# vitasoftAI/ImageRetrievalResearch

Measured on AMD Instinct MI355X. Metric: images/sec embed + queries/sec top-k@100k-gallery, EffNet-B3a 224^2, higher is better.
Workload: dtype bf16

## Files before the change

### imageretrievalresearch_amd/csrc/mbconv_block.hip

```cpp
#include "ops.h"

namespace mi355 {

typedef __bf16 bf16x8 __attribute__((ext_vector_type(8)));
typedef float f32x4 __attribute__((ext_vector_type(4)));
typedef unsigned u32x4 __attribute__((ext_vector_type(4)));
typedef unsigned u32x2 __attribute__((ext_vector_type(2)));

constexpr int MB_THREADS = 512;
constexpr int MB_WAVES = MB_THREADS / 64;
constexpr int MB_MAX_RD = 192;
constexpr int MB_MC = MB_WAVES * 16;

__device__ __forceinline__ float mb_lo(unsigned u) { return __uint_as_float(u << 16); }
__device__ __forceinline__ float mb_hi(unsigned u) { return __uint_as_float(u & 0xffff0000u); }

__device__ __forceinline__ void mb_lds_barrier() {
    asm volatile("s_waitcnt lgkmcnt(0)" ::: "memory");
    __builtin_amdgcn_s_barrier();
    asm volatile("" ::: "memory");
}

__host__ __device__ static inline int mb_proj_ntw(int NTp, int MTp, int NTW) {
    int best = 1, best_busy = 0;
// ... 12 lines not shown
    const int ntw = mb_proj_ntw(NTp, MTp, 3);
    if (wi != 14) return ntw;
    const int nwn = (NTp + ntw - 1) / ntw;
    int msplit = nwn <= MB_WAVES ? MB_WAVES / nwn : 1;
    if (msplit > MTp) msplit = MTp;
    if (nwn <= MB_WAVES && (MTp + msplit - 1) / msplit <= mwp) return ntw;
    return 4;
}

template <int KS> struct MbTaps {
    static constexpr int KK = KS * KS;
    static constexpr int NV = (KS / 2) * KS;
    static constexpr int NH = (KS + 1) / 2;
    static constexpr int NP = NV + NH;
    __host__ __device__ static constexpr bool vertical(int tp) { return tp < NV; }
    __host__ __device__ static constexpr int tap_a(int tp) {
        return tp < NV ? (tp / KS) * 2 * KS + tp % KS : (KS - 1) * KS + (tp - NV) * 2;
    }
    __host__ __device__ static constexpr int tap_b(int tp) {
        return tp < NV ? tap_a(tp) + KS : ((tp - NV) * 2 + 1 < KS ? tap_a(tp) + 1 : -1);
    }
};

template <int KS, int S, int WI, int MW, int MH, int NTW, int MWP, int KST, int A_IT, int ACT_E, int ACT_D>
__global__ __launch_bounds__(MB_THREADS) void k_mbconv_block(const BlockArgs a) {
    using TP = MbTaps<KS>;
    constexpr int MC = MB_MC;
    constexpr int PAD = KS / 2;
    constexpr int NP = TP::NP;
    constexpr int EW = WI + 2 * PAD;
    constexpr int WO = (WI + 2 * PAD - KS) / S + 1;
    constexpr int TR = WO <= 8 ? 2 : 1;
    constexpr int RP = (TR == 2 && S == 1) ? ((EW + 7) & ~7) : EW;
    static_assert(WO <= 16, "depthwise tile geometry");
    constexpr bool PROJ_WHOLE = WI == 7 && NTW == 2;
    constexpr int KC = WI == 7 ? 256 : 128;
    constexpr int ALD = KC + 16;
    extern __shared__ __attribute__((aligned(16))) unsigned char mb_smem[];

    const int tid = threadIdx.x, lane = tid & 63;
    const int wave = __builtin_amdgcn_readfirstlane(tid >> 6);
    const int fr = lane & 15, fq = lane >> 4, fk = fq * 8;
    const int b = blockIdx.x;
    const int P = a.H * a.W, MT = (P + 15) >> 4, XLD = a.XLD;
    const int EH = a.H + 2 * PAD;
    const int EP = (EH + (TR == 2 ? S : 0)) * RP + 8;
    const int Pout = a.Ho * a.Wo;
// ... 24 lines not shown
    u32x4 wq[KST];
    f32x4 be_reg;
    auto w_prefetch_slab = [&](int cbase) {
        const int n = min(cbase + wave * 16 + fr, midp - 1);
#pragma unroll
        for (int h = 0; h < KST; ++h) wq[h] = *reinterpret_cast<const u32x4*>(a.We + (n * a.Kp + fk + h * 32));
        be_reg = *reinterpret_cast<const f32x4*>(a.be + min(cbase + wave * 16 + fq * 4, midp - 4));
        __builtin_amdgcn_sched_barrier(0);
    };
    unsigned short wd_raw[NP], wd_nxt[NP];
    f32x4 bd_reg, bd_nxt;
    auto wd_fetch = [&](int cbase) {
        const int ch = min(cbase + wave * 16 + fr, a.mid - 1);
#pragma unroll
        for (int tp = 0; tp < NP; ++tp) {
            const int ta = TP::tap_a(tp), tb = TP::tap_b(tp) < 0 ? TP::tap_a(tp) : TP::tap_b(tp);
            const int t = (lane & 32) ? tb : ta;
            wd_nxt[tp] = a.Wd[t * a.mid + ch];
        }
        bd_nxt = *reinterpret_cast<const f32x4*>(a.bd + min(cbase + wave * 16 + fq * 4, a.mid - 4));
        __builtin_amdgcn_sched_barrier(0);
    };

    w_prefetch_slab(slab_of(0) * MC);
    wd_fetch(slab_of(0) * MC);
    {
        const int kc = (a.Cin + 7) >> 3;
        const int kcl = XLD >> 3;
        const bf16_t* xb = a.X + (size_t)b * P * a.Cin;
        const int total = MT * 16 * kcl;
        constexpr int U = 9;
        for (int id0 = tid; id0 < total; id0 += MB_THREADS * U) {
            u32x4 v[U];
            int dst[U];
#pragma unroll
            for (int u = 0; u < U; ++u) {
                const int id = id0 + u * MB_THREADS;
                const int row = id / kcl, c = id - row * kcl;
                const u32x4 t = *reinterpret_cast<const u32x4*>(xb + (min(row, P - 1) * a.Cin + min(c, kc - 1) * 8));
                const bool ok = id < total && row < P && c < kc;
                v[u] = ok ? t : (u32x4){0u, 0u, 0u, 0u};
                dst[u] = id < total ? row * XLD + c * 8 : -1;
            }
            if (id0 == tid) {
                bf16_t* Eall = reinterpret_cast<bf16_t*>(R);
                for (int id = tid; id < MB_WAVES * EP * 2; id += MB_THREADS)
                    *reinterpret_cast<u32x4*>(&Eall[id * 8]) = (u32x4){0u, 0u, 0u, 0u};
                if (tid < 4) *reinterpret_cast<u32x4*>(&Xs[MT * 16 * XLD + tid * 8]) = (u32x4){0u, 0u, 0u, 0u};
            }
#pragma unroll
            for (int u = 0; u < U; ++u)
                if (dst[u] >= 0) *reinterpret_cast<u32x4*>(&Xs[dst[u]]) = v[u];
        }
    }
    mb_lds_barrier();
    tick(0);

    bf16_t* Db = a.D + (size_t)b * Pout * a.mid;

    const int e_cv = (fq & 1) * 8 + ((fq >> 1) ? RP * 16 : 0);
    const int e_ch = (fq & 1) * 8 + ((fq >> 1) ? 16 : 0);
    const int t_row = TR == 2 ? (fr >> 3) : 0, t_col = TR == 2 ? (fr & 7) : fr;
    const int e_lane = (t_row * S * RP + t_col * S) * 16;
    constexpr int E_TILE = TR * S * RP * 16;
    const bool col_ok = t_col < WO;

    const int abl = a.variant;
    bool prev_active = false;
    for (int ci = 0; ci < nslabs; ++ci) {
        const int cbase = slab_of(ci) * MC;
        const int ch0 = cbase + wave * 16;
        const bool active = ch0 < a.mid;
        {
            constexpr int MTO_SQ = TR == 2 ? (WO + 1) / 2 : WO;
            if (ci > 0 && prev_active && MTo == MTO_SQ) {
                if constexpr (MTO_SQ >= 14) asm volatile("s_waitcnt vmcnt(14)" ::: "memory");
                else if constexpr (MTO_SQ >= 4) asm volatile("s_waitcnt vmcnt(4)" ::: "memory");
                else asm volatile("s_waitcnt vmcnt(1)" ::: "memory");
            } else {
                asm volatile("s_waitcnt vmcnt(0)" ::: "memory");
            }
#pragma unroll
            for (int h = 0; h < KST; ++h) asm volatile("" : "+v"(wq[h]));
            asm volatile("" : "+v"(be_reg));
            asm volatile("" : "+v"(bd_nxt));
#pragma unroll
            for (int tp = 0; tp < NP; ++tp) { asm volatile("" : "+v"(wd_nxt[tp])); wd_raw[tp] = wd_nxt[tp]; }
            bd_reg = bd_nxt;
        }
        tick(1);
// ... 89 lines not shown
                }
                acc.x = act_c<ACT_D>(acc.x); acc.y = act_c<ACT_D>(acc.y); acc.z = act_c<ACT_D>(acc.z); acc.w = act_c<ACT_D>(acc.w);
                if (col_ok && mt * TR + t_row < a.Ho) {
                    psum[0] += acc.x; psum[1] += acc.y; psum[2] += acc.z; psum[3] += acc.w;
                    if (chok) {
                        u32x2 ov;
                        ov.x = pack2bf(acc.x, acc.y);
                        ov.y = pack2bf(acc.z, acc.w);
                        *reinterpret_cast<u32x2*>(dlane + mt * d_tile) = ov;
                    }
                }
            }
#pragma unroll
            for (int o = 1; o < 16; o <<= 1) {
#pragma unroll
                for (int j = 0; j < 4; ++j) psum[j] += __shfl_xor(psum[j], o, 64);
            }
            if (fr == 0 && chok)
                *reinterpret_cast<f32x4*>(&pool[ch0 + fq * 4]) = (f32x4){psum[0], psum[1], psum[2], psum[3]};
        }
        prev_active = active;
        tick(2);
        asm volatile("" ::: "memory");
    }
    constexpr int C8MAX = 5;
    const int ngroups = (abl & 4) ? 0 : (a.rd + 3) >> 2;
    auto fc1_load = [&](int gi, u32x4 (&w)[C8MAX][4], float (&b1v)[4]) {
        const int j0 = ((gi + rb1) % max(ngroups, 1)) * 4;
#pragma unroll
        for (int it = 0; it < C8MAX; ++it) {
            const int c8 = min(lane + it * 64, (a.mid >> 3) - 1);
#pragma unroll
            for (int q = 0; q < 4; ++q)
                w[it][q] = *reinterpret_cast<const u32x4*>(a.W1 + (min(j0 + q, a.rd - 1) * a.mid + c8 * 8));
        }
#pragma unroll
        for (int q = 0; q < 4; ++q) b1v[q] = a.b1[min(j0 + q, a.rd - 1)];
        __builtin_amdgcn_sched_barrier(0);
    };
    auto fc1_compute = [&](int gi, const u32x4 (&w)[C8MAX][4], const float (&b1v)[4]) {
        const int j0 = ((gi + rb1) % max(ngroups, 1)) * 4;
        float s[4] = {0.f, 0.f, 0.f, 0.f};
#pragma unroll
        for (int it = 0; it < C8MAX; ++it) {
            const int c8 = lane + it * 64;
            if (c8 * 8 < a.mid) {
// ... 427 lines not shown
    if (act_e != ACT_SILU) return false;
    if (Cin % 8 || mid % 8 || mid > 2560 || Cout % 8 || rd < 1 || rd > MB_MAX_RD) return false;
    if (!((k == 3 || k == 5) && (stride == 1 || stride == 2))) return false;
    if (W == 7 && stride == 2) return false;
    if ((long)mid * ((Cin + 31) & ~31) >= (1l << 30) || (long)Cout * mid >= (1l << 30)) return false;
    BlockArgs a{};
    a.H = H; a.W = W; a.Cin = Cin; a.Kp = (Cin + 31) & ~31; a.mid = mid; a.Cout = Cout;
    const int pad = k / 2;
    a.Ho = (H + 2 * pad - k) / stride + 1; a.Wo = (W + 2 * pad - k) / stride + 1;
    const int Pout = a.Ho * a.Wo, MTp = (Pout + 15) / 16, NTp = (Cout + 15) / 16;
    const int ntw = mb_pick_ntw(NTp, MTp, g.wi, g.mwp);
    const int nwn = (NTp + ntw - 1) / ntw;
    if (nwn > MB_WAVES) return false;
    int msplit = MB_WAVES / nwn;
    if (msplit > MTp) msplit = MTp;
    if ((MTp + msplit - 1) / msplit > g.mwp) return false;
    a.Kp2 = (mid + 31) & ~31;
    if (Pout * (g.wi == 7 ? 32 : 16) > g.a_it * MB_THREADS) return false;
    if ((H * W + 15) / 16 > g.mw * g.mh) return false;
    if (!mb_instance_ok(k, stride, g.wi, a.Kp / 32, ntw, act_d)) return false;
    return mb_pick_xld(a, k, g) != 0;
}

template <int KS, int S, int WI, int MW, int MH, int NTW, int MWP, int KST, int A_IT, int ACT_E, int ACT_D>
static int launch_mb(BlockArgs a, int B, hipStream_t st) {
    MbGeom g;
    mb_geom(a.H, a.W, &g);
    a.XLD = mb_pick_xld(a, KS, g);
    a.KCS = mb_pick_kcs(a);
    const size_t lds = mb_lds_bytes_xld(a, KS, a.XLD, g);
    static bool attr_done[64] = {false};
    int dev = 0;
    MI355_CHECK_HIP(hipGetDevice(&dev));
    if (dev >= 0 && dev < 64 && !attr_done[dev]) {
        MI355_CHECK_HIP(hipFuncSetAttribute((const void*)k_mbconv_block<KS, S, WI, MW, MH, NTW, MWP, KST, A_IT, ACT_E, ACT_D>,
                                            hipFuncAttributeMaxDynamicSharedMemorySize, 160 * 1024));
        attr_done[dev] = true;
    }
    hipLaunchKernelGGL((k_mbconv_block<KS, S, WI, MW, MH, NTW, MWP, KST, A_IT, ACT_E, ACT_D>), dim3(B), dim3(MB_THREADS), lds, st, a);
    MI355_LAUNCH_CHECK();
    return OK;
}

int launch_mbconv_block(const BlockArgs& a, int B, int k, int stride, hipStream_t st) {
    MI355_REQUIRE(mbconv_block_supported(a.H, a.W, a.Cin, a.mid, a.Cout, k, stride, a.rd, a.act_e, a.act_d), "mbconv_block: unsupported shape");
    const int Pout = a.Ho * a.Wo;
    MbGeom gg;
    mb_geom(a.H, a.W, &gg);
    const int ntw = mb_pick_ntw((a.Cout + 15) / 16, (Pout + 15) / 16, gg.wi, gg.mwp);
    const int kst = a.Kp / 32;
#define X(KS, S, WI, KST, NTW, AD)                                                                  \
    if (k == KS && stride == S && a.W == WI && kst == KST && ntw == NTW && a.act_d == AD)           \
        return launch_mb<KS, S, WI, (WI == 7 ? 4 : 7), (WI == 7 ? 1 : 2), NTW, (WI == 7 ? 4 : 7), KST, (WI == 7 ? 4 : 7), ACT_SILU, AD>(a, B, st);
    MB_INSTANCES(X)
#undef X
    set_error("mbconv_block: no instance for k=%d s=%d W=%d Kp=%d ntw=%d", k, stride, a.W, a.Kp, ntw);
    return ERR_UNSUPPORTED;
}

}
```

### imageretrievalresearch_amd/csrc/model.hip

```cpp
#include "model_exec.h"
#include "../../include/mi355_retrieval.h"

#include <string.h>

#include <algorithm>

namespace mi355 {

int pack_gemm(Packer& pk, Op& op) {
    const TensorSpec* w = pk.get(op.w_name);
    if (!w) return ERR_STATE;
    const int N = op.cout_real, K = op.cin_real;
    MI355_REQUIRE(w->numel() == (int64_t)N * K, "pack: %s has %lld elements, expected %d x %d", op.w_name.c_str(),
                  (long long)w->numel(), N, K);
    std::vector<float> scale, shift;
    if (!pk.bn_fold(op.bn_name, op.bn_eps, N, scale, shift)) return ERR_STATE;
    if (!op.bias_name.empty()) {
        const TensorSpec* b = pk.get(op.bias_name);
        if (!b) return ERR_STATE;
        for (int i = 0; i < N; ++i) shift[i] = b->data[i] * scale[i] + shift[i];
    }
    const int Np = (op.cout + 15) & ~15, Kp = (op.cin + 31) & ~31;
    op.w_off = pk.alloc((size_t)Np * Kp * 2);
    op.b_off = pk.alloc((size_t)Np * 4);
// ... 302 lines not shown
    if (g.kind != OP_GEMM || d.kind != OP_DW || g.out != SLOT_E || d.in != SLOT_E) return false;
    if (g.use_gate || g.res != SLOT_NONE || g.a_relu6 || !g.tap.empty()) return false;
    if (fused_late_supported(h, w, g.cin, g.cout, d.k, d.stride)) return true;
    if (use_sweep(m, g, d, h, w)) return true;
    const int rows = m->fuse_band ? fused_band_rows(h, w, g.cin, g.cout, d.k, d.stride) : 0;
    const bool measured_win = d.k == 3 && ((d.stride == 1 && rows >= 7) || (d.stride == 2 && w >= 112 && g.cout >= 192));
    return rows > 0 && (m->fuse_band == 1 || measured_win);
}

static bool can_fuse_block(const mi355_model* m, size_t i, int h, int w, int nb) {
    if (!m->fuse_block || nb < m->fuse_block_min_batch || i + 3 >= m->def.ops.size()) return false;
    const Op& g = m->def.ops[i];
    const Op& d = m->def.ops[i + 1];
    const Op& s = m->def.ops[i + 2];
    const Op& p = m->def.ops[i + 3];
    if (g.kind != OP_GEMM || d.kind != OP_DW || s.kind != OP_SE || p.kind != OP_GEMM) return false;
    if (g.out != SLOT_E || d.in != SLOT_E || d.out != SLOT_D || p.in != SLOT_D || !p.use_gate || !d.pool) return false;
    if (g.use_gate || g.res != SLOT_NONE || g.a_relu6 || !g.tap.empty() || !d.tap.empty()) return false;
    if (p.act != ACT_NONE || (p.res != SLOT_NONE && p.res != g.in)) return false;
    if (p.res != SLOT_NONE && p.res_channels && ((p.res_channels + 7) & ~7) != g.cin) return false;
    return mbconv_block_supported(h, w, g.cin, g.cout, p.cout, d.k, d.stride, s.rd, g.act, d.act);
}

static int stamp_ptr(ExecCtx& cx, size_t oi, long long** out) {
    mi355_model* m = cx.m;
    *out = nullptr;
    if (!m->block_stamps) return OK;
    const size_t need = m->def.ops.size() * (size_t)cx.B * 16 * sizeof(long long);
    if (m->stamp_bytes < need) {
        if (m->stamp_buf) MI355_CHECK_HIP(hipFree(m->stamp_buf));
        MI355_CHECK_HIP(hipMalloc((void**)&m->stamp_buf, need));
        m->stamp_bytes = need;
    }
    m->stamp_B = cx.B;
    *out = m->stamp_buf + (oi * (size_t)cx.B + cx.b0) * 16;
    MI355_CHECK_HIP(hipMemsetAsync(*out, 0, (size_t)cx.nb * 16 * sizeof(long long), cx.st));
    return OK;
}

static int exec_block(ExecCtx& cx, size_t oi) {
    mi355_model* m = cx.m;
    SlotState* S = m->slots;
    const Op& g = m->def.ops[oi];
    const Op& d = m->def.ops[oi + 1];
    const Op& s = m->def.ops[oi + 2];
    const Op& p = m->def.ops[oi + 3];
    BlockArgs a{};
    a.X = (const bf16_t*)cx.slot_ptr(g.in);
    a.We = (const bf16_t*)cx.w(g.w_off); a.be = (const float*)cx.w(g.b_off);
    a.Wd = (const bf16_t*)cx.w(d.w_off); a.bd = (const float*)cx.w(d.b_off);
    a.W1 = (const bf16_t*)cx.w(s.w3_off); a.b1 = (const float*)cx.w(s.b_off);
    a.W2 = (const bf16_t*)cx.w(s.w4_off); a.b2 = (const float*)cx.w(s.b2_off);
    a.Wp = (const bf16_t*)cx.w(p.w_off); a.bp = (const float*)cx.w(p.b_off);
    a.D = (bf16_t*)cx.slot_ptr(d.out);
    a.Y = (bf16_t*)cx.slot_ptr(p.out);
    a.H = S[g.in].h; a.W = S[g.in].w; a.Cin = g.cin; a.Kp = (g.cin + 31) & ~31; a.mid = g.cout;
    a.Ho = S[d.out].h; a.Wo = S[d.out].w; a.Cout = p.cout; a.Kp2 = (p.cin + 31) & ~31; a.rd = s.rd;
    a.has_res = p.res != SLOT_NONE;
    a.res_n = p.res != SLOT_NONE ? (p.res_channels ? ((p.res_channels + 7) & ~7) : p.cout) : 0;
    a.a_relu6 = p.a_relu6;
    a.act_e = g.act; a.act_d = d.act; a.se_act = s.se_act;
    a.inv_hw = 1.0f / (float)(a.Ho * a.Wo);
    a.norot = m->block_norot;
    a.variant = m->block_variant;
    a.stamps = nullptr;
    { const int rc = stamp_ptr(cx, oi, &a.stamps); if (rc != OK) return rc; }
    return launch_mbconv_block(a, cx.nb, d.k, d.stride, cx.st);
}

static int exec_fused(ExecCtx& cx, const Op& g, const Op& d) {
    mi355_model* m = cx.m;
    SlotState* S = m->slots;
    FusedArgs a{};
    a.X = (const bf16_t*)cx.slot_ptr(g.in);
    a.We = (const bf16_t*)cx.w(g.w_off); a.be = (const float*)cx.w(g.b_off);
    a.Wd = (const bf16_t*)cx.w(d.w_off); a.bd = (const float*)cx.w(d.b_off);
    a.D = (bf16_t*)cx.slot_ptr(d.out);
    a.pool = d.pool ? (float*)cx.slot_ptr(SLOT_POOLPART) : nullptr;
    a.H = S[g.in].h; a.W = S[g.in].w; a.Cin = g.cin; a.Kp = (g.cin + 31) & ~31; a.mid = g.cout;
    a.Ho = S[d.out].h; a.Wo = S[d.out].w; a.act_e = g.act; a.act_d = d.act;
    a.debug_skip = m->fuse_debug;
    if (fused_late_supported(a.H, a.W, g.cin, g.cout, d.k, d.stride)) {
        m->pool_nblk = 1;
        return launch_fused_late(a, cx.nb, d.k, d.stride, cx.st);
    }
    if (use_sweep(m, g, d, a.H, a.W)) {
        SweepArgs sa{};
        sa.X = a.X; sa.We = a.We; sa.be = a.be; sa.Wd = a.Wd; sa.bd = a.bd; sa.D = a.D; sa.pool = a.pool;
// ... 8 lines not shown
    return launch_fused_band(a, cx.nb, d.k, d.stride, cx.st);
}

static void op_range_label(const Op& op, int H, int W, int in_h, int in_w, const char* how, char* lab, size_t n) {
    switch (op.kind) {
        case OP_STEM: snprintf(lab, n, "embed/%sstem 3->%d @%dx%d", how, op.cout_real, conv_out(H, 3, 2), conv_out(W, 3, 2)); break;
        case OP_GEMM: snprintf(lab, n, "embed/%spw %d->%d @%dx%d%s%s", how, op.cin_real, op.cout_real, in_h, in_w,
                               op.use_gate ? " gate" : "", op.res != SLOT_NONE ? " res" : ""); break;
        case OP_DW: snprintf(lab, n, "embed/%sdw k%d s%d C%d @%dx%d", how, op.k, op.stride, op.cin_real, in_h, in_w); break;
        case OP_SE: snprintf(lab, n, "embed/%sse C%d rd%d", how, op.cin_real, op.rd); break;
        default: snprintf(lab, n, "embed/%sop%d C%d->%d t%d", how, (int)op.kind, op.cin_real, op.cout_real, op.tokens_h); break;
    }
}

static int run_backbone(ExecCtx& cx, size_t op_begin = 0, size_t op_end = (size_t)-1) {
    mi355_model* m = cx.m;
    SlotState* S = m->slots;
    if (op_end > m->def.ops.size()) op_end = m->def.ops.size();
    for (size_t oi = op_begin; oi < op_end; ++oi) {
        const Op& op = m->def.ops[oi];
        const int op_index = (int)oi;
        const int in_h = S[op.in == SLOT_NONE ? 0 : op.in].h, in_w = S[op.in == SLOT_NONE ? 0 : op.in].w;
        const bool block = op.in != SLOT_NONE && can_fuse_block(m, oi, in_h, in_w, cx.B);
        const bool fused = block || can_fuse(m, oi, in_h, in_w);
        if (fused) {
            const Op& d = m->def.ops[oi + 1];
            S[op.out].h = S[op.in].h; S[op.out].w = S[op.in].w; S[op.out].c = op.cout;
            S[d.out].h = conv_out(S[op.in].h, d.k, d.stride); S[d.out].w = conv_out(S[op.in].w, d.k, d.stride);
            S[d.out].c = d.cout;
            if (block) {
                const Op& pj = m->def.ops[oi + 3];
                S[pj.out].h = S[d.out].h; S[pj.out].w = S[d.out].w; S[pj.out].c = pj.cout;
            }
        } else
        switch (op.kind) {
            case OP_STEM: S[op.out].h = conv_out(cx.H, 3, 2); S[op.out].w = conv_out(cx.W, 3, 2); S[op.out].c = op.cout; break;
            case OP_GEMM: S[op.out].h = S[op.in].h; S[op.out].w = S[op.in].w; S[op.out].c = op.cout; break;
            case OP_DW: {
                const int ho = conv_out(S[op.in].h, op.k, op.stride), wo = conv_out(S[op.in].w, op.k, op.stride);
                S[op.out].h = ho; S[op.out].w = wo; S[op.out].c = op.cout;
                break;
            }
            case OP_SE: break;
            default: if (op.out != SLOT_NONE) { S[op.out].h = op.tokens_h; S[op.out].w = op.tokens_h; S[op.out].c = op.cout; } break;
        }
        hipEvent_t e0 = nullptr, e1 = nullptr;
        if (m->profile) {
            MI355_CHECK_HIP(hipEventCreate(&e0));
            MI355_CHECK_HIP(hipEventCreate(&e1));
            MI355_CHECK_HIP(hipEventRecord(e0, cx.st));
        }
        {
            char lab[192] = "";
            if (roctx_active())
                op_range_label(op, cx.H, cx.W, in_h, in_w, block ? "block: " : (fused ? "fused: " : ""), lab, sizeof lab);
            RoctxRange range(lab);
            if (block) {
                if (int e = exec_block(cx, oi)) return e;
            } else if (fused) {
                if (int e = exec_fused(cx, op, m->def.ops[oi + 1])) return e;
            } else if (int e = exec_op(cx, op)) return e;
        }
        if (m->profile) {
            MI355_CHECK_HIP(hipEventRecord(e1, cx.st));
            m->prof_events.push_back({op_index, {e0, e1}});
            if (m->prof_fused.size() < m->def.ops.size()) m->prof_fused.resize(m->def.ops.size(), 0);
            m->prof_fused[op_index] = fused ? 1 : 0;
        }
        if (block) {
            const Op& pj = m->def.ops[oi + 3];
            if (m->taps && !pj.tap.empty())
                if (int e = record_tap(cx, pj)) return e;
            oi += 3;
            continue;
        }
        if (m->taps && !op.tap.empty())
            if (int e = record_tap(cx, op)) return e;
        if (fused) ++oi;
    }
    return OK;
}

struct U8Source {
    const unsigned char* img = nullptr;
    const int64_t* desc = nullptr;
    int h = 0, w = 0, fill = 255;
    float mean[3] = {0.f, 0.f, 0.f}, stdv[3] = {1.f, 1.f, 1.f};
    const float* conv_w = nullptr;
};

// ... 337 lines not shown
    auto it = m->tapbufs.find(tap_name);
    MI355_REQUIRE(it != m->tapbufs.end(), "read_tap: no tap named '%s' was recorded", tap_name);
    const TapBuf& t = it->second;
    if (shape) { shape[0] = t.B; shape[1] = t.c_real; shape[2] = t.h; shape[3] = t.w; }
    if (!out) return OK;
    MI355_REQUIRE(out_numel >= (int64_t)t.B * t.c_real * t.h * t.w, "read_tap: output too small");
    return launch_nhwc_to_nchw_f32((const bf16_t*)t.ptr, out, t.B, t.h * t.w, t.c, t.c_real, (hipStream_t)stream);
}

int mi355_model_set_option(mi355_model_t m, const char* key, int64_t value) {
    MI355_REQUIRE(m && key, "set_option: null argument");
    const std::string k = key;
    if (k == "microbatch") m->microbatch = (int)value;
    else if (k == "lanes") m->lanes = (int)value;
    else if (k == "fuse") m->fuse = value != 0;
    else if (k == "fuse_band") m->fuse_band = (int)value;
    else if (k == "fuse_sweep") m->fuse_sweep = (int)value;
    else if (k == "sweep_csplit") m->sweep_csplit = (int)value;
    else if (k == "sweep_variant") m->sweep_variant = (int)value;
    else if (k == "sweep_skip") m->sweep_skip = (int)value;
    else if (k == "fuse_debug") m->fuse_debug = (int)value;
    else if (k == "fuse_ln") m->fuse_ln = (int)value;
    else if (k == "fuse_block") m->fuse_block = (int)value;
    else if (k == "fuse_block_min_batch") m->fuse_block_min_batch = (int)value;
    else if (k == "block_stamps") m->block_stamps = value != 0;
    else if (k == "block_norot") m->block_norot = (int)value;
    else if (k == "block_variant") m->block_variant = (int)value;
    else if (k == "fuse_head_gap") m->fuse_head_gap = value != 0;
    else if (k == "roctx") roctx_enable(value != 0);
    else if (k == "profile") {
        m->profile = value != 0;
        for (int i = 0; i < PK_COUNT; ++i) { m->prof_ms[i] = 0; m->prof_launches[i] = 0; }
        m->prof_op_ms.assign(m->def.ops.size(), 0.0);
        m->prof_op_n.assign(m->def.ops.size(), 0);
    } else {
        set_error("set_option: unknown option '%s'", key);
        return ERR_ARG;
    }
    return OK;
}

int mi355_model_profile_read(mi355_model_t m, double* ms_by_kind, int64_t* launches_by_kind, int n) {
    MI355_REQUIRE(m && ms_by_kind && launches_by_kind && n >= PK_COUNT, "profile_read: need arrays of >= %d", PK_COUNT);
    for (auto& pe : m->prof_events) {
        MI355_CHECK_HIP(hipEventSynchronize(pe.second.second));
        float ms = 0.f;
// ... 299 lines not shown
```

### imageretrievalresearch_amd/csrc/model_exec.h

```cpp
#pragma once
#include "model.h"

#include <string.h>

namespace mi355 {

int swin_exec(const ModelDef& def, const Op& op, struct ExecCtx& cx);

static inline uint16_t f2bf_host(float f) {
    uint32_t u;
    memcpy(&u, &f, 4);
    if ((u & 0x7fffffffu) > 0x7f800000u) return (uint16_t)((u >> 16) | 0x40);
    u += 0x7fffu + ((u >> 16) & 1u);
    return (uint16_t)(u >> 16);
}
static inline float bf_round_host(float f) {
    uint32_t u = ((uint32_t)f2bf_host(f)) << 16;
    float r;
    memcpy(&r, &u, 4);
    return r;
}

struct SlotState {
    size_t off = 0, bytes = 0;
// ... 14 lines not shown

struct mi355_model {
    ModelDef def;
    std::vector<char> blob;
    void* dev_blob = nullptr;
    size_t dev_blob_bytes = 0;
    bool packed = false;
    void* arena = nullptr;
    size_t arena_bytes = 0;
    int arena_device = -1, blob_device = -1;
    SlotState slots[SLOT_COUNT];
    int microbatch = 0;
    int lanes = 1;
    hipStream_t lane_stream[4] = {nullptr, nullptr, nullptr, nullptr};
    hipEvent_t lane_fork = nullptr, lane_join[4] = {nullptr, nullptr, nullptr, nullptr};
    size_t lane_bytes = 0;
    int fuse_sweep = 1;
    int sweep_variant = 0, sweep_skip = 0;
    int sweep_csplit = 0;
    int fuse_band = 2;
    bool fuse = true;
    int fuse_block = 1;
    int fuse_block_min_batch = 96;
    bool fuse_head_gap = true;
    int block_variant = 0;
    int block_norot = 0;
    bool block_stamps = false;
    long long* stamp_buf = nullptr; size_t stamp_bytes = 0; int stamp_B = 0;
    int fuse_debug = 0;
    int fuse_ln = 1;
    int pool_nblk = 0;
    bool taps = false;
    std::map<std::string, TapBuf> tapbufs;
    bool profile = false;
    std::vector<std::pair<int, std::pair<hipEvent_t, hipEvent_t>>> prof_events;
    std::vector<char> prof_fused;
    std::vector<double> prof_op_ms;
    std::vector<long> prof_op_n;
    double prof_ms[PK_COUNT] = {0};
    long prof_launches[PK_COUNT] = {0};
};

namespace mi355 {

struct ExecCtx {
    mi355_model* m;
// ... 51 lines not shown
```

### imageretrievalresearch_amd/csrc/ops.h

```cpp
#pragma once
#include "common.h"

namespace mi355 {

struct GemmArgs {
    const bf16_t* A; int lda;
    const bf16_t* W; int ldw;
    const float* bias;
    const bf16_t* res; int ldr; int res_n;
    const float* gate; int gate_ld; int rows_per_img;
    void* out; int ldo; int out_f32;
    int M, N, K;
    int act;
    int a_relu6;
    const bf16_t* zeros;
    long M_sel;
    float* splitk_ws;
    size_t splitk_ws_bytes;
    const float* ln_stats;
    const float* ln_colsum;
};
int launch_gemm_bf16(const GemmArgs& a, hipStream_t st, int* path = nullptr);
bool gemm_wide_supported(const GemmArgs& a);
int launch_gemm_wide(const GemmArgs& a, hipStream_t st);
// ... 27 lines not shown
    bf16_t* D;
    float* pool;
    int B, H, W, Cin, Kp, mid, Ho, Wo;
    int act_e, act_d;
    int csplit;
    int csplit_override;
    int variant;
    int debug_skip;
    long long* stamps;
};
bool sweep_mbconv_supported(int H, int W, int Cin, int mid, int k, int stride, int act_e, int act_d);
int launch_sweep_mbconv(const SweepArgs& a, int B, int k, int stride, hipStream_t st);

struct BlockArgs {
    const bf16_t* X;
    const bf16_t* We; const float* be;
    const bf16_t* Wd; const float* bd;
    const bf16_t* W1; const float* b1;
    const bf16_t* W2; const float* b2;
    const bf16_t* Wp; const float* bp;
    bf16_t* D;
    bf16_t* Y;
    long long* stamps;
    int H, W, Cin, Kp, mid, Ho, Wo, Cout, Kp2, rd;
    int XLD;
    int KCS;
    int norot;
    int variant;
    int has_res;
    int res_n;
    int a_relu6;
    int act_e, act_d, se_act;
    float inv_hw;
};
bool mbconv_block_supported(int H, int W, int Cin, int mid, int Cout, int k, int stride, int rd, int act_e, int act_d);
int launch_mbconv_block(const BlockArgs& a, int B, int k, int stride, hipStream_t st);

int launch_stem(const float* x, const float* w, const float* bias, bf16_t* out, int B, int H, int W, int Cout,
                int act, hipStream_t st);

int launch_stem_u8(const unsigned char* img, int h, int w, int fill, const float* mean, const float* stdv,
                   const float* conv_w, const float* sw, const float* bias, bf16_t* out, int B, int Cout, int act,
                   hipStream_t st, const int64_t* desc = nullptr, int b0 = 0);

int check_images(const unsigned char* pixels, int64_t pixels_bytes, const int64_t* desc_host, const int64_t* desc_dev, int B,
                 const char* who);
size_t resize_batch_workspace(const int64_t* desc_host, int B, int out_h, int out_w, bool pad);
int resize_batch(const unsigned char* pixels, int64_t pixels_bytes, const int64_t* desc_host, const int64_t* desc_dev, int B,
                 int out_h, int out_w, bool pad, int fill, unsigned char* out, void* workspace, size_t workspace_bytes,
                 hipStream_t st);

int dw_pool_blocks(int Ho, int Wo, int C);
int launch_dwconv(const bf16_t* in, const bf16_t* w, const float* bias, bf16_t* out, float* pool_partial, int B,
                  int H, int W, int C, int k, int stride, int act, int* pool_nblk, hipStream_t st);
int launch_dwconv_sel(const bf16_t* in, const bf16_t* w, const float* bias, bf16_t* out, float* pool_partial, int B,
                      int H, int W, int C, int k, int stride, int act, bool try_tiled, bool try_mfma, int* pool_nblk,
                      int* path, hipStream_t st);
void dw_env_choice(bool* try_tiled, bool* try_mfma);
bool dw_tiled_supported(int H, int W, int C, int k, int stride);
// ... 24 lines not shown
```

Before: 62440.

## Split 7x7 MBConv blocks into multi-image front kernel plus SE/project back kernel

```diff
diff --git a/imageretrievalresearch_amd/csrc/mbconv_block.hip b/imageretrievalresearch_amd/csrc/mbconv_block.hip
--- a/imageretrievalresearch_amd/csrc/mbconv_block.hip
+++ b/imageretrievalresearch_amd/csrc/mbconv_block.hip
@@ -58,7 +58,7 @@
     }
 };
 
-template <int KS, int S, int WI, int MW, int MH, int NTW, int MWP, int KST, int A_IT, int ACT_E, int ACT_D>
+template <int KS, int S, int WI, int MW, int MH, int NTW, int MWP, int KST, int A_IT, int ACT_E, int ACT_D, bool BACK = false>
 __global__ __launch_bounds__(MB_THREADS) void k_mbconv_block(const BlockArgs a) {
     using TP = MbTaps<KS>;
     constexpr int MC = MB_MC;
@@ -129,6 +129,12 @@
         __builtin_amdgcn_sched_barrier(0);
     };
 
+    bf16_t* Db = a.D + (size_t)b * Pout * a.mid;
+    const int abl = a.variant;
+    if constexpr (BACK) {
+        const float* sqb = a.sq + (size_t)b * a.mid;
+        for (int c = tid * 4; c < a.mid; c += MB_THREADS * 4) *reinterpret_cast<f32x4*>(&pool[c]) = *reinterpret_cast<const f32x4*>(&sqb[c]);
+    } else {
     w_prefetch_slab(slab_of(0) * MC);
     wd_fetch(slab_of(0) * MC);
     {
@@ -163,8 +169,6 @@
     mb_lds_barrier();
     tick(0);
 
-    bf16_t* Db = a.D + (size_t)b * Pout * a.mid;
-
     const int e_cv = (fq & 1) * 8 + ((fq >> 1) ? RP * 16 : 0);
     const int e_ch = (fq & 1) * 8 + ((fq >> 1) ? 16 : 0);
     const int t_row = TR == 2 ? (fr >> 3) : 0, t_col = TR == 2 ? (fr & 7) : fr;
@@ -172,7 +176,6 @@
     constexpr int E_TILE = TR * S * RP * 16;
     const bool col_ok = t_col < WO;
 
-    const int abl = a.variant;
     bool prev_active = false;
     for (int ci = 0; ci < nslabs; ++ci) {
         const int cbase = slab_of(ci) * MC;
@@ -308,6 +311,7 @@
         prev_active = active;
         tick(2);
         asm volatile("" ::: "memory");
+    }
     }
     constexpr int C8MAX = 5;
     const int ngroups = (abl & 4) ? 0 : (a.rd + 3) >> 2;
@@ -781,7 +785,7 @@
     return mb_pick_xld(a, k, g) != 0;
 }
 
-template <int KS, int S, int WI, int MW, int MH, int NTW, int MWP, int KST, int A_IT, int ACT_E, int ACT_D>
+template <int KS, int S, int WI, int MW, int MH, int NTW, int MWP, int KST, int A_IT, int ACT_E, int ACT_D, bool BACK = false>
 static int launch_mb(BlockArgs a, int B, hipStream_t st) {
     MbGeom g;
     mb_geom(a.H, a.W, &g);
@@ -792,11 +796,11 @@
     int dev = 0;
     MI355_CHECK_HIP(hipGetDevice(&dev));
     if (dev >= 0 && dev < 64 && !attr_done[dev]) {
-        MI355_CHECK_HIP(hipFuncSetAttribute((const void*)k_mbconv_block<KS, S, WI, MW, MH, NTW, MWP, KST, A_IT, ACT_E, ACT_D>,
+        MI355_CHECK_HIP(hipFuncSetAttribute((const void*)k_mbconv_block<KS, S, WI, MW, MH, NTW, MWP, KST, A_IT, ACT_E, ACT_D, BACK>,
                                             hipFuncAttributeMaxDynamicSharedMemorySize, 160 * 1024));
         attr_done[dev] = true;
     }
-    hipLaunchKernelGGL((k_mbconv_block<KS, S, WI, MW, MH, NTW, MWP, KST, A_IT, ACT_E, ACT_D>), dim3(B), dim3(MB_THREADS), lds, st, a);
+    hipLaunchKernelGGL((k_mbconv_block<KS, S, WI, MW, MH, NTW, MWP, KST, A_IT, ACT_E, ACT_D, BACK>), dim3(B), dim3(MB_THREADS), lds, st, a);
     MI355_LAUNCH_CHECK();
     return OK;
 }
@@ -817,4 +821,35 @@
     return ERR_UNSUPPORTED;
 }
 
-}
+#define MB_BACK_INSTANCES(X) X(5, 1, 7, 8, 2, ACT_SILU) X(3, 1, 7, 8, 3, ACT_SILU) X(3, 1, 7, 12, 3, ACT_SILU)
+bool mbconv_block_back_supported(int H, int W, int Cin, int mid, int Cout, int k, int stride, int rd, int act_e, int act_d) {
+    if (!mbconv_block_supported(H, W, Cin, mid, Cout, k, stride, rd, act_e, act_d)) return false;
+    MbGeom g;
+    mb_geom(H, W, &g);
+    const int pad = k / 2;
+    const int Pout = ((H + 2 * pad - k) / stride + 1) * ((W + 2 * pad - k) / stride + 1);
+    const int ntw = mb_pick_ntw((Cout + 15) / 16, (Pout + 15) / 16, g.wi, g.mwp), kst = ((Cin + 31) & ~31) / 32;
+#define X(KS, S, WI, KST, NTW, AD) if (k == KS && stride == S && g.wi == WI && kst == KST && ntw == NTW && act_d == AD) return true;
+    MB_BACK_INSTANCES(X)
+#undef X
+    return false;
+}
+
+int launch_mbconv_block_back(const BlockArgs& a, int B, int k, int stride, hipStream_t st) {
+    MI355_REQUIRE(a.sq && mbconv_block_back_supported(a.H, a.W, a.Cin, a.mid, a.Cout, k, stride, a.rd, a.act_e, a.act_d),
+                  "mbconv_block_back: unsupported shape");
+    const int Pout = a.Ho * a.Wo;
+    MbGeom gg;
+    mb_geom(a.H, a.W, &gg);
+    const int ntw = mb_pick_ntw((a.Cout + 15) / 16, (Pout + 15) / 16, gg.wi, gg.mwp);
+    const int kst = a.Kp / 32;
+#define X(KS, S, WI, KST, NTW, AD)                                                                  \
+    if (k == KS && stride == S && a.W == WI && kst == KST && ntw == NTW && a.act_d == AD)           \
+        return launch_mb<KS, S, WI, 4, 1, NTW, 4, KST, 4, ACT_SILU, AD, true>(a, B, st);
+    MB_BACK_INSTANCES(X)
+#undef X
+    set_error("mbconv_block_back: no instance for k=%d s=%d W=%d Kp=%d ntw=%d", k, stride, a.W, a.Kp, ntw);
+    return ERR_UNSUPPORTED;
+}
+
+}
diff --git a/imageretrievalresearch_amd/csrc/mbconv_group.hip b/imageretrievalresearch_amd/csrc/mbconv_group.hip
--- /dev/null
+++ b/imageretrievalresearch_amd/csrc/mbconv_group.hip
@@ -0,0 +1,305 @@
+#include "ops.h"
+
+#include <type_traits>
+
+namespace mi355 {
+
+typedef __bf16 bf16x8 __attribute__((ext_vector_type(8)));
+typedef float f32x4 __attribute__((ext_vector_type(4)));
+typedef unsigned u32x4 __attribute__((ext_vector_type(4)));
+typedef unsigned u32x2 __attribute__((ext_vector_type(2)));
+
+constexpr int MG_THREADS = 512;
+constexpr int MG_WAVES = MG_THREADS / 64;
+constexpr int MG_P = 49;
+constexpr int MG_BD_BYTES = 4608;
+
+template <int KS> struct MgTaps {
+    static constexpr int NV = (KS / 2) * KS;
+    static constexpr int NH = (KS + 1) / 2;
+    static constexpr int NP = NV + NH;
+    __host__ __device__ static constexpr bool vertical(int tp) { return tp < NV; }
+    __host__ __device__ static constexpr int tap_a(int tp) {
+        return tp < NV ? (tp / KS) * 2 * KS + tp % KS : (KS - 1) * KS + (tp - NV) * 2;
+    }
+    __host__ __device__ static constexpr int tap_b(int tp) {
+        return tp < NV ? tap_a(tp) + KS : ((tp - NV) * 2 + 1 < KS ? tap_a(tp) + 1 : -1);
+    }
+};
+
+template <int KS, int KST> struct MgGeom {
+    static constexpr int PAD = KS / 2;
+    static constexpr int EW = 7 + 2 * PAD;
+    static constexpr int RP = (EW + 7) & ~7;
+    static constexpr int EH = 7 + 2 * PAD;
+    static constexpr int EP = (EH + 1) * RP + 8;
+    static constexpr int XLD = KST * 32 + 16;
+    __host__ __device__ static constexpr size_t x_bytes(int nimg) { return ((size_t)nimg * MG_P * XLD * 2 + 15) & ~(size_t)15; }
+    __host__ __device__ static constexpr size_t e_bytes() { return (size_t)MG_WAVES * EP * 16 * 2; }
+    __host__ __device__ static constexpr size_t lds_bytes(int nimg) { return x_bytes(nimg) + e_bytes() + MG_BD_BYTES; }
+};
+
+template <int KS, int NIMG, int KST>
+__global__ __launch_bounds__(MG_THREADS) void k_mbconv_group_front(const BlockArgs a, const int nb) {
+    using TP = MgTaps<KS>;
+    using G = MgGeom<KS, KST>;
+    constexpr int PAD = G::PAD, NP = TP::NP, RP = G::RP, EP = G::EP, XLD = G::XLD;
+    constexpr int WI = 7, WO = 7, MW = 4, MTO = 4;
+    constexpr int ACT_E = ACT_SILU, ACT_D = ACT_SILU;
+    extern __shared__ __attribute__((aligned(16))) unsigned char mg_smem[];
+
+    const int tid = threadIdx.x, lane = tid & 63;
+    const int wave = __builtin_amdgcn_readfirstlane(tid >> 6);
+    const int fr = lane & 15, fq = lane >> 4, fk = fq * 8;
+    const int q = blockIdx.x, part = blockIdx.y;
+    const int midp = (a.mid + 15) & ~15;
+    const int NT = midp >> 4;
+    const int t0 = NT * part / NIMG, t1 = NT * (part + 1) / NIMG;
+    const int nslabs = (t1 - t0 + MG_WAVES - 1) / MG_WAVES;
+
+    bf16_t* Xs = reinterpret_cast<bf16_t*>(mg_smem);
+    unsigned char* R = mg_smem + G::x_bytes(NIMG);
+    bf16_t* Es = reinterpret_cast<bf16_t*>(R) + (size_t)wave * EP * 16;
+    float* Bds = reinterpret_cast<float*>(R + G::e_bytes());
+
+    auto tile_of = [&](int ci) { return t0 + ((ci + q) % nslabs) * MG_WAVES + wave; };
+
+    u32x4 wq[KST];
+    f32x4 be_reg;
+    unsigned wd_raw[NP], wd_nxt[NP];
+    f32x4 bd_reg;
+    auto w_prefetch = [&](int tile) {
+        const int n = min(tile * 16 + fr, midp - 1);
+#pragma unroll
+        for (int h = 0; h < KST; ++h) wq[h] = *reinterpret_cast<const u32x4*>(a.We + (n * a.Kp + fk + h * 32));
+        be_reg = *reinterpret_cast<const f32x4*>(a.be + min(tile * 16 + fq * 4, midp - 4));
+        const int ch = min(tile * 16 + fr, a.mid - 1);
+#pragma unroll
+        for (int tp = 0; tp < NP; ++tp) {
+            const int ta = TP::tap_a(tp), tb = TP::tap_b(tp) < 0 ? TP::tap_a(tp) : TP::tap_b(tp);
+            const int t = (lane & 32) ? tb : ta;
+            wd_nxt[tp] = (unsigned)a.Wd[t * a.mid + ch];
+        }
+        __builtin_amdgcn_sched_barrier(0);
+    };
+
+    w_prefetch(tile_of(0));
+    {
+        const int kc = a.Cin >> 3;
+        constexpr int kcl = XLD >> 3;
+        constexpr int total = NIMG * MG_P * kcl;
+        bf16_t* Eall = reinterpret_cast<bf16_t*>(R);
+        for (int id = tid; id < MG_WAVES * EP * 2; id += MG_THREADS)
+            *reinterpret_cast<u32x4*>(&Eall[id * 8]) = (u32x4){0u, 0u, 0u, 0u};
+        for (int i = tid; i < (t1 - t0) * 16; i += MG_THREADS) Bds[i] = a.bd[min(t0 * 16 + i, a.mid - 1)];
+        constexpr int U = 7;
+        for (int id0 = tid; id0 < total; id0 += MG_THREADS * U) {
+            u32x4 v[U];
+            int dst[U];
+#pragma unroll
+            for (int u = 0; u < U; ++u) {
+                const int id = min(id0 + u * MG_THREADS, total - 1);
+                const int row = id / kcl, c = id - row * kcl;
+                const int img = row / MG_P, p = row - img * MG_P;
+                const int bi = min(q * NIMG + img, nb - 1);
+                const u32x4 t = *reinterpret_cast<const u32x4*>(a.X + (((size_t)bi * MG_P + p) * a.Cin + min(c, kc - 1) * 8));
+                v[u] = c < kc ? t : (u32x4){0u, 0u, 0u, 0u};
+                dst[u] = id0 + u * MG_THREADS < total ? row * XLD + c * 8 : -1;
+            }
+#pragma unroll
+            for (int u = 0; u < U; ++u)
+                if (dst[u] >= 0) *reinterpret_cast<u32x4*>(&Xs[dst[u]]) = v[u];
+        }
+    }
+    asm volatile("s_waitcnt lgkmcnt(0)" ::: "memory");
+    __builtin_amdgcn_s_barrier();
+    asm volatile("" ::: "memory");
+
+    const int e_cv = (fq & 1) * 8 + ((fq >> 1) ? RP * 16 : 0);
+    const int e_ch = (fq & 1) * 8 + ((fq >> 1) ? 16 : 0);
+    const int t_row = fr >> 3, t_col = fr & 7;
+    const int e_lane = (t_row * RP + t_col) * 16;
+    constexpr int E_TILE = 2 * RP * 16;
+    const bool col_ok = t_col < WO;
+    int arow[MW];
+#pragma unroll
+    for (int i = 0; i < MW; ++i) arow[i] = min(i * 16 + fr, MG_P - 1) * XLD + fk;
+
+    bool prev_stores = false;
+#pragma nounroll
+    for (int ci = 0; ci < nslabs; ++ci) {
+        const int tile = tile_of(ci);
+        const int ch0 = tile * 16;
+        const bool active = tile < t1;
+        if (ci > 0 && prev_stores) asm volatile("s_waitcnt vmcnt(4)" ::: "memory");
+        else asm volatile("s_waitcnt vmcnt(0)" ::: "memory");
+#pragma unroll
+        for (int h = 0; h < KST; ++h) asm volatile("" : "+v"(wq[h]));
+        asm volatile("" : "+v"(be_reg));
+#pragma unroll
+        for (int tp = 0; tp < NP; ++tp) { asm volatile("" : "+v"(wd_nxt[tp])); wd_raw[tp] = wd_nxt[tp]; }
+        bd_reg = *reinterpret_cast<const f32x4*>(&Bds[(min(tile, t1 - 1) - t0) * 16 + fq * 4]);
+        const bool has_next = ci + 1 < nslabs;
+        const int tile_next = tile_of(has_next ? ci + 1 : ci);
+
+        auto do_image = [&](auto IC) {
+            constexpr int img = decltype(IC)::value;
+            const int bi = q * NIMG + img;
+            const bool valid = bi < nb;
+            const bf16_t* Xi = Xs + img * MG_P * XLD;
+            f32x4 acc[MW];
+#pragma unroll
+            for (int i = 0; i < MW; ++i) acc[i] = be_reg;
+            constexpr int PD = 2;
+            bf16x8 af[PD + 1][MW];
+#pragma unroll
+            for (int d = 0; d < PD; ++d)
+#pragma unroll
+                for (int i = 0; i < MW; ++i) af[d][i] = *reinterpret_cast<const bf16x8*>(&Xi[arow[i] + (d < KST ? d : KST - 1) * 32]);
+            if (active) {
+#pragma unroll
+                for (int ks = 0; ks < KST; ++ks) {
+                    if (ks + PD < KST) {
+#pragma unroll
+                        for (int i = 0; i < MW; ++i)
+                            af[(ks + PD) % (PD + 1)][i] = *reinterpret_cast<const bf16x8*>(&Xi[arow[i] + (ks + PD) * 32]);
+                    }
+#pragma unroll
+                    for (int i = 0; i < MW; ++i)
+                        acc[i] = __builtin_amdgcn_mfma_f32_16x16x32_bf16(*reinterpret_cast<bf16x8*>(&wq[ks]), af[ks % (PD + 1)][i], acc[i], 0, 0, 0);
+                }
+            }
+            if constexpr (img == NIMG - 1) {
+                if (has_next) w_prefetch(tile_next);
+            }
+            if (active) {
+#pragma unroll
+                for (int i = 0; i < MW; ++i) {
+                    acc[i].x = act_c<ACT_E>(acc[i].x); acc[i].y = act_c<ACT_E>(acc[i].y);
+                    acc[i].z = act_c<ACT_E>(acc[i].z); acc[i].w = act_c<ACT_E>(acc[i].w);
+                }
+#pragma unroll
+                for (int i = 0; i < MW; ++i) {
+                    const int p = i * 16 + fr;
+                    if (p < MG_P) {
+                        const int y = p / WI;
+                        const int eoff = (y + PAD) * RP + (p - y * WI) + PAD;
+                        u32x2 o;
+                        o.x = pack2bf(acc[i].x, acc[i].y);
+                        o.y = pack2bf(acc[i].z, acc[i].w);
+                        *reinterpret_cast<u32x2*>(&Es[eoff * 16 + fq * 4]) = o;
+                    }
+                }
+            }
+            asm volatile("" ::: "memory");
+            if (active && valid) {
+                u32x4 dwf[NP];
+                {
+                    const bool mine = ((fq & 1) == (fr >> 3)) && (ch0 + fr < a.mid);
+#pragma unroll
+                    for (int tp = 0; tp < NP; ++tp) {
+                        const bool has = mine && !((lane & 32) && TP::tap_b(tp) < 0);
+                        const unsigned v = has ? wd_raw[tp] : 0u;
+                        const unsigned word = (fr & 1) ? (v << 16) : v;
+                        const int qq = (fr & 7) >> 1;
+                        dwf[tp] = (u32x4){qq == 0 ? word : 0u, qq == 1 ? word : 0u, qq == 2 ? word : 0u, qq == 3 ? word : 0u};
+                    }
+                }
+                auto e_read = [&](int tbase, int tp) -> bf16x8 {
+                    const int ta = TP::tap_a(tp);
+                    const int offs = ((ta / KS) * RP + (ta % KS)) * 16;
+                    return *reinterpret_cast<const bf16x8*>(Es + tbase + (TP::vertical(tp) ? e_cv : e_ch) + offs);
+                };
+                bf16x8 ef[NP];
+#pragma unroll
+                for (int tp = 0; tp < NP; ++tp) ef[tp] = e_read(e_lane, tp);
+                float psum[4] = {0.f, 0.f, 0.f, 0.f};
+                const bool chok = ch0 + fq * 4 < a.mid;
+                bf16_t* dlane = a.D + (size_t)bi * MG_P * a.mid + ((t_row * WO + t_col) * a.mid + ch0 + fq * 4);
+                const size_t d_tile = (size_t)2 * WO * a.mid;
+                for (int mt = 0; mt < MTO; ++mt) {
+                    const int tbn = e_lane + min(mt + 1, MTO - 1) * E_TILE;
+                    f32x4 dacc = bd_reg;
+#pragma unroll
+                    for (int tp = 0; tp < NP; ++tp) {
+                        dacc = __builtin_amdgcn_mfma_f32_16x16x32_bf16(*reinterpret_cast<bf16x8*>(&dwf[tp]), ef[tp], dacc, 0, 0, 0);
+                        ef[tp] = e_read(tbn, tp);
+                    }
+                    dacc.x = act_c<ACT_D>(dacc.x); dacc.y = act_c<ACT_D>(dacc.y); dacc.z = act_c<ACT_D>(dacc.z); dacc.w = act_c<ACT_D>(dacc.w);
+                    if (col_ok && mt * 2 + t_row < WO) {
+                        psum[0] += dacc.x; psum[1] += dacc.y; psum[2] += dacc.z; psum[3] += dacc.w;
+                        if (chok) {
+                            u32x2 ov;
+                            ov.x = pack2bf(dacc.x, dacc.y);
+                            ov.y = pack2bf(dacc.z, dacc.w);
+                            *reinterpret_cast<u32x2*>(dlane + mt * d_tile) = ov;
+                        }
+                    }
+                }
+#pragma unroll
+                for (int o = 1; o < 16; o <<= 1) {
+#pragma unroll
+                    for (int j = 0; j < 4; ++j) psum[j] += __shfl_xor(psum[j], o, 64);
+                }
+                if (fr == 0 && chok)
+                    *reinterpret_cast<f32x4*>(a.sq + (size_t)bi * a.mid + ch0 + fq * 4) = (f32x4){psum[0], psum[1], psum[2], psum[3]};
+            }
+            if constexpr (img == NIMG - 1) prev_stores = active && valid;
+            asm volatile("" ::: "memory");
+        };
+        do_image(std::integral_constant<int, 0>{});
+        do_image(std::integral_constant<int, 1>{});
+        if constexpr (NIMG == 4) {
+            do_image(std::integral_constant<int, 2>{});
+            do_image(std::integral_constant<int, 3>{});
+        }
+    }
+}
+
+#define MG_INSTANCES(X) X(5, 8, 4) X(3, 8, 4) X(3, 12, 2)
+
+bool mbconv_group_supported(int H, int W, int Cin, int mid, int Cout, int k, int stride, int rd, int act_e, int act_d) {
+    if (H != 7 || W != 7 || stride != 1 || act_e != ACT_SILU || act_d != ACT_SILU || mid % 16 || Cin % 8) return false;
+    if (!mbconv_block_back_supported(H, W, Cin, mid, Cout, k, stride, rd, act_e, act_d)) return false;
+    const int kst = ((Cin + 31) & ~31) / 32;
+#define X(KS, KST, NI) \
+    if (k == KS && kst == KST) return MgGeom<KS, KST>::lds_bytes(NI) <= 160 * 1024 && (mid / 16 + NI - 1) / NI * 64 <= MG_BD_BYTES;
+    MG_INSTANCES(X)
+#undef X
+    return false;
+}
+
+template <int KS, int NIMG, int KST>
+static int launch_front(const BlockArgs& a, int B, hipStream_t st) {
+    constexpr size_t lds = MgGeom<KS, KST>::lds_bytes(NIMG);
+    static_assert(lds <= 160 * 1024, "mbconv_group: X and the E images do not fit the LDS");
+    static bool attr_done[64] = {false};
+    int dev = 0;
+    MI355_CHECK_HIP(hipGetDevice(&dev));
+    if (dev >= 0 && dev < 64 && !attr_done[dev]) {
+        MI355_CHECK_HIP(hipFuncSetAttribute((const void*)k_mbconv_group_front<KS, NIMG, KST>,
+                                            hipFuncAttributeMaxDynamicSharedMemorySize, 160 * 1024));
+        attr_done[dev] = true;
+    }
+    hipLaunchKernelGGL((k_mbconv_group_front<KS, NIMG, KST>), dim3((B + NIMG - 1) / NIMG, NIMG), dim3(MG_THREADS), lds, st, a, B);
+    MI355_LAUNCH_CHECK();
+    return OK;
+}
+
+int launch_mbconv_group(const BlockArgs& a, int B, int k, int stride, hipStream_t st, int phase) {
+    MI355_REQUIRE(B >= 1 && a.sq && a.D && mbconv_group_supported(a.H, a.W, a.Cin, a.mid, a.Cout, k, stride, a.rd, a.act_e, a.act_d),
+                  "mbconv_group: unsupported shape");
+    MI355_REQUIRE((long)B * MG_P * a.mid < (1l << 31) && a.Kp == ((a.Cin + 31) & ~31), "mbconv_group: bad arguments");
+    if (phase != 2) {
+        const int kst = a.Kp / 32;
+        int rc = ERR_UNSUPPORTED;
+#define X(KS, KST, NI) if (k == KS && kst == KST) rc = launch_front<KS, NI, KST>(a, B, st);
+        MG_INSTANCES(X)
+#undef X
+        if (rc != OK) return rc;
+    }
+    if (phase != 1) return launch_mbconv_block_back(a, B, k, stride, st);
+    return OK;
+}
+
+}
diff --git a/imageretrievalresearch_amd/csrc/model.hip b/imageretrievalresearch_amd/csrc/model.hip
--- a/imageretrievalresearch_amd/csrc/model.hip
+++ b/imageretrievalresearch_amd/csrc/model.hip
@@ -348,6 +348,18 @@
     return mbconv_block_supported(h, w, g.cin, g.cout, p.cout, d.k, d.stride, s.rd, g.act, d.act);
 }
 
+static bool can_group_block(const mi355_model* m, size_t i, int h, int w, int nb) {
+    if (!m->fuse_group || m->block_stamps || m->block_variant || !can_fuse_block(m, i, h, w, nb)) return false;
+    const Op& g = m->def.ops[i];
+    const Op& d = m->def.ops[i + 1];
+    const Op& s = m->def.ops[i + 2];
+    const Op& p = m->def.ops[i + 3];
+    if (p.a_relu6) return false;
+    if (!mbconv_group_supported(h, w, g.cin, g.cout, p.cout, d.k, d.stride, s.rd, g.act, d.act)) return false;
+    const bool level = g.cin == 232 && p.cout == 384;
+    return m->fuse_group == 2 || !level;
+}
+
 static int stamp_ptr(ExecCtx& cx, size_t oi, long long** out) {
     mi355_model* m = cx.m;
     *out = nullptr;
@@ -364,7 +376,7 @@
     return OK;
 }
 
-static int exec_block(ExecCtx& cx, size_t oi) {
+static int exec_block(ExecCtx& cx, size_t oi, int group_phase = -1) {
     mi355_model* m = cx.m;
     SlotState* S = m->slots;
     const Op& g = m->def.ops[oi];
@@ -390,6 +402,10 @@
     a.norot = m->block_norot;
     a.variant = m->block_variant;
     a.stamps = nullptr;
+    if (group_phase >= 0) {
+        a.sq = (float*)cx.slot_ptr(SLOT_POOLPART);
+        return launch_mbconv_group(a, cx.nb, d.k, d.stride, cx.st, group_phase);
+    }
     { const int rc = stamp_ptr(cx, oi, &a.stamps); if (rc != OK) return rc; }
     return launch_mbconv_block(a, cx.nb, d.k, d.stride, cx.st);
 }
@@ -444,6 +460,7 @@
         const int op_index = (int)oi;
         const int in_h = S[op.in == SLOT_NONE ? 0 : op.in].h, in_w = S[op.in == SLOT_NONE ? 0 : op.in].w;
         const bool block = op.in != SLOT_NONE && can_fuse_block(m, oi, in_h, in_w, cx.B);
+        const bool group = block && can_group_block(m, oi, in_h, in_w, cx.B);
         const bool fused = block || can_fuse(m, oi, in_h, in_w);
         if (fused) {
             const Op& d = m->def.ops[oi + 1];
@@ -478,7 +495,7 @@
                 op_range_label(op, cx.H, cx.W, in_h, in_w, block ? "block: " : (fused ? "fused: " : ""), lab, sizeof lab);
             RoctxRange range(lab);
             if (block) {
-                if (int e = exec_block(cx, oi)) return e;
+                if (int e = exec_block(cx, oi, group ? (m->profile ? 1 : 0) : -1)) return e;
             } else if (fused) {
                 if (int e = exec_fused(cx, op, m->def.ops[oi + 1])) return e;
             } else if (int e = exec_op(cx, op)) return e;
@@ -488,6 +505,15 @@
             m->prof_events.push_back({op_index, {e0, e1}});
             if (m->prof_fused.size() < m->def.ops.size()) m->prof_fused.resize(m->def.ops.size(), 0);
             m->prof_fused[op_index] = fused ? 1 : 0;
+            if (group) {
+                hipEvent_t f0 = nullptr, f1 = nullptr;
+                MI355_CHECK_HIP(hipEventCreate(&f0));
+                MI355_CHECK_HIP(hipEventCreate(&f1));
+                MI355_CHECK_HIP(hipEventRecord(f0, cx.st));
+                if (int e = exec_block(cx, oi, 2)) return e;
+                MI355_CHECK_HIP(hipEventRecord(f1, cx.st));
+                m->prof_events.push_back({op_index + 3, {f0, f1}});
+            }
         }
         if (block) {
             const Op& pj = m->def.ops[oi + 3];
@@ -871,6 +897,7 @@
     else if (k == "fuse_debug") m->fuse_debug = (int)value;
     else if (k == "fuse_ln") m->fuse_ln = (int)value;
     else if (k == "fuse_block") m->fuse_block = (int)value;
+    else if (k == "fuse_group") m->fuse_group = (int)value;
     else if (k == "fuse_block_min_batch") m->fuse_block_min_batch = (int)value;
     else if (k == "block_stamps") m->block_stamps = value != 0;
     else if (k == "block_norot") m->block_norot = (int)value;
diff --git a/imageretrievalresearch_amd/csrc/model_exec.h b/imageretrievalresearch_amd/csrc/model_exec.h
--- a/imageretrievalresearch_amd/csrc/model_exec.h
+++ b/imageretrievalresearch_amd/csrc/model_exec.h
@@ -60,6 +60,7 @@
     bool fuse = true;
     int fuse_block = 1;
     int fuse_block_min_batch = 96;
+    int fuse_group = 1;
     bool fuse_head_gap = true;
     int block_variant = 0;
     int block_norot = 0;
diff --git a/imageretrievalresearch_amd/csrc/ops.h b/imageretrievalresearch_amd/csrc/ops.h
--- a/imageretrievalresearch_amd/csrc/ops.h
+++ b/imageretrievalresearch_amd/csrc/ops.h
@@ -73,6 +73,7 @@
     bf16_t* D;
     bf16_t* Y;
     long long* stamps;
+    float* sq;
     int H, W, Cin, Kp, mid, Ho, Wo, Cout, Kp2, rd;
     int XLD;
     int KCS;
@@ -86,6 +87,11 @@
 };
 bool mbconv_block_supported(int H, int W, int Cin, int mid, int Cout, int k, int stride, int rd, int act_e, int act_d);
 int launch_mbconv_block(const BlockArgs& a, int B, int k, int stride, hipStream_t st);
+bool mbconv_block_back_supported(int H, int W, int Cin, int mid, int Cout, int k, int stride, int rd, int act_e, int act_d);
+int launch_mbconv_block_back(const BlockArgs& a, int B, int k, int stride, hipStream_t st);
+
+bool mbconv_group_supported(int H, int W, int Cin, int mid, int Cout, int k, int stride, int rd, int act_e, int act_d);
+int launch_mbconv_group(const BlockArgs& a, int B, int k, int stride, hipStream_t st, int phase = 0);
 
 int launch_stem(const float* x, const float* w, const float* bias, bf16_t* out, int B, int H, int W, int Cout,
                 int act, hipStream_t st);
```

Result: no change. 62300 (median of 4 runs) (-0.2%).
